# qianlim/CAPE

Hardware: NVIDIA B200
Metric: meshes/sec fwd+bwd CAPE-affineconv nz64 (higher is better)
Workload: dtype f32

## Files before the change

### cape_b200/_lib.py

```python
import ctypes as C
import os

_HERE = os.path.dirname(os.path.abspath(__file__))
LIB_PATH = os.environ.get("CAPE_B200_LIB") or os.path.join(_HERE, "libcape_b200.so")

MAX_TERMS = 8
EPI_LINEAR, EPI_AFFINE, EPI_SLOPE, EPI_DUALMASK = 0, 1, 2, 3
ACT_NONE, ACT_LEAKY, ACT_RELU = 0, 1, 2

f32p = C.c_void_p


class Term(C.Structure):
    _fields_ = [("src", C.c_void_p), ("op", C.c_int), ("F", C.c_int), ("src_rows", C.c_int),
                ("src_stride", C.c_int), ("w_stride", C.c_int), ("w2_stride", C.c_int), ("w", C.c_void_p), ("w2", C.c_void_p),
                ("wc", C.c_void_p), ("wc2", C.c_void_p), ("wT", C.c_void_p), ("w2T", C.c_void_p),
                ("wT_stride", C.c_int), ("w2T_stride", C.c_int), ("stash", C.c_void_p), ("stash_stride", C.c_int),
                ("wT_lo", C.c_void_p), ("w2T_lo", C.c_void_p)]


class ConvArgs(C.Structure):
    _fields_ = [("N", C.c_int), ("rows_out", C.c_int), ("ncols", C.c_int), ("nterms", C.c_int),
                ("terms", Term * MAX_TERMS), ("cond", C.c_void_p), ("C", C.c_int), ("epilogue", C.c_int),
                ("act", C.c_int), ("alpha", C.c_float), ("bias", C.c_void_p), ("bias_per_row", C.c_int),
# ... 29 lines not shown
                ("F", C.c_int), ("src_rows", C.c_int), ("src_stride", C.c_int), ("g", C.c_void_p),
                ("dw", C.c_void_p), ("dw_stride", C.c_int), ("accumulate", C.c_int), ("nops", C.c_int),
                ("ops", C.c_int * MAX_TERMS), ("dw_term_stride", C.c_int), ("dw_col_stride", C.c_int)]


SIGNATURES = {
    "cape_last_error": (C.c_char_p, []),
    "cape_abi_version": (C.c_int, []),
    "cape_launch_count": (C.c_int64, []),
    "cape_topology_create": (C.c_int, [C.c_int, C.POINTER(C.c_void_p)]),
    "cape_topology_destroy": (None, [C.c_void_p]),
    "cape_topology_add_operator": (C.c_int, [C.c_void_p, C.c_int, C.c_int, C.c_int, C.c_void_p, C.c_void_p]),
    "cape_topology_reserve_workspace": (C.c_int, [C.c_void_p, C.c_int64]),
    "cape_set_tensor_cores": (C.c_int, [C.c_int]),
    "cape_tensor_cores_enabled": (C.c_int, []),
    "cape_gemm_batch": (C.c_int, [C.c_void_p, C.c_int, C.c_void_p, C.c_int, C.c_void_p]),
    "cape_gemm_item_bytes": (C.c_int, []),
    "cape_gather_rows": (C.c_int, [C.c_void_p, C.c_int64, C.c_int, C.c_void_p, C.c_int, C.c_void_p, C.c_void_p]),
    "cape_weight_prep": (C.c_int, [C.c_void_p, C.c_int, C.c_int, C.c_void_p]),
    "cape_set_tuning": (C.c_int, [C.c_int, C.c_int]),
    "cape_cheb_fwd": (C.c_int, [C.c_void_p, C.POINTER(ConvArgs), C.c_void_p]),
    "cape_apply": (C.c_int, [C.c_void_p, C.POINTER(ApplyArgs), C.c_void_p]),
    "cape_cheb_dw": (C.c_int, [C.c_void_p, C.POINTER(DwArgs), C.c_void_p]),
    "cape_colsum": (C.c_int, [C.c_void_p, C.c_void_p, C.c_int, C.c_int, C.c_int, C.c_int, C.POINTER(C.c_int), C.c_int,
                              C.c_void_p, C.c_void_p]),
    "cape_gemm": (C.c_int, [C.c_void_p, C.c_int, C.c_int, C.c_int, C.c_void_p, C.c_int64, C.c_int64, C.c_void_p,
                            C.c_int64, C.c_int64, C.c_void_p, C.c_int64, C.c_void_p, C.c_int, C.c_float, C.c_float,
                            C.c_float, C.c_void_p]),
    "cape_resample": (C.c_int, [C.c_void_p, C.c_int, C.c_void_p, C.c_int, C.c_void_p, C.c_int, C.c_int, C.c_int, C.c_int,
                                C.c_int, C.c_void_p, C.c_int, C.c_void_p]),
    "cape_cheb_weight_transpose": (C.c_int, [C.c_void_p, C.c_int, C.c_int, C.c_int, C.c_void_p, C.c_void_p, C.c_void_p]),
    "cape_tf32_lo": (C.c_int, [C.c_void_p, C.c_void_p, C.c_int64, C.c_void_p]),
    "cape_act_bwd": (C.c_int, [C.c_void_p, C.c_void_p, C.c_void_p, C.c_int64, C.c_float, C.c_void_p]),
    "cape_axpy": (C.c_int, [C.c_void_p, C.c_void_p, C.c_float, C.c_int64, C.c_void_p]),
    "cape_vae_sample_fwd": (C.c_int, [C.c_void_p, C.c_void_p, C.c_void_p, C.c_void_p, C.c_int, C.c_int, C.c_int,
                                      C.c_void_p]),
    "cape_vae_sample_bwd": (C.c_int, [C.c_void_p, C.c_int, C.c_void_p, C.c_void_p, C.c_void_p, C.c_void_p,
                                      C.c_void_p, C.c_int, C.c_int, C.c_float, C.c_void_p]),
    "cape_recon_losses": (C.c_int, [C.c_void_p, C.c_int, C.c_void_p, C.c_void_p, C.c_int, C.c_int, C.c_float,
                                    C.c_float, C.c_int, C.c_void_p, C.c_void_p, C.c_int, C.c_void_p, C.c_void_p,
                                    C.c_void_p]),
    "cape_bce_logits": (C.c_int, [C.c_void_p, C.c_int64, C.c_float, C.c_float, C.c_void_p, C.c_void_p, C.c_void_p]),
    "cape_sumsq": (C.c_int, [C.c_void_p, C.c_int64, C.c_void_p, C.c_void_p]),
    "cape_sgd_clip_update": (C.c_int, [C.c_void_p, C.c_void_p, C.c_void_p, C.c_int64, C.c_void_p, C.c_float,
                                       C.c_void_p, C.c_float, C.c_void_p]),
    "cape_adam_clip_update": (C.c_int, [C.c_void_p, C.c_void_p, C.c_void_p, C.c_void_p, C.c_int64, C.c_void_p, C.c_float,
# ... 35 lines not shown
```

### cape_b200/csrc/dw_dense_tma.cu

```cuda
#include "common.cuh"
#include "ellconv_params.cuh"
#include "tc_common.cuh"

namespace cape {

namespace {

using namespace tc;

constexpr int DD_CONV_WARPS = 8;
constexpr int DD_CONV_THREADS = DD_CONV_WARPS * 32;
constexpr int DD_THREADS = DD_CONV_THREADS + 64;
constexpr int DD_KCH = 32;
constexpr int DD_A_TILE = 4 * 4096;
constexpr int DD_MAX_STAGES = 8;
constexpr int DD_SMEM_BUDGET = 212 * 1024;

struct DdParams {
  int ncols, F;
  long long total_rows, rows_per_split;
  float* out;
  long long out_rs;
  int nsplit, accumulate, ovec, lo_mode;
  int sah, sal, sgh, sgl;
  int budget;
};

template <int BN>
struct DdCfg {
  static constexpr int G_TILE = (BN / 32) * 4096;
  static constexpr int SMEM_BYTES = 1024 + DD_SMEM_BUDGET + 1024;
};

template <int BN>
void dd_plan(int nct, DdParams* p) {
  constexpr int GT = DdCfg<BN>::G_TILE;
  p->sal = 2; p->sgl = 2;
  int left = p->budget - 2 * DD_A_TILE - 2 * GT;
  int sah = nct >= 2 ? 3 : 2, sgh = 2;
  left -= sah * DD_A_TILE + sgh * GT;
  while (true) {
    const bool to_g = (sgh < DD_MAX_STAGES) && ((long long)sgh < (long long)sah * nct || sah >= DD_MAX_STAGES);
    const int cost = to_g ? GT : DD_A_TILE;
    if ((to_g ? sgh : sah) >= DD_MAX_STAGES || cost > left) break;
    left -= cost;
    if (to_g) ++sgh; else ++sah;
  }
  p->sah = sah; p->sgh = sgh;
// ... 40 lines not shown
  if (warp == DD_CONV_WARPS) {
    if (lane == 0) {
      for (int s = 0; s < DD_MAX_STAGES; ++s) {
        mbar_init(bar_ahf + 8 * s, 1); mbar_init(bar_ahe + 8 * s, 1);
        mbar_init(bar_alf + 8 * s, DD_CONV_WARPS); mbar_init(bar_ale + 8 * s, 1);
        mbar_init(bar_ghf + 8 * s, 1); mbar_init(bar_ghe + 8 * s, 1);
        mbar_init(bar_glf + 8 * s, DD_CONV_WARPS); mbar_init(bar_gle + 8 * s, 1);
      }
      mbar_init(bar_accum, 1);
      fence_mbar_init();
    }
    __syncwarp();
    tmem_alloc(smem_u32(tmem_slot), (uint32_t)tmem_cols);
  }
  tc_fence_before();
  __syncthreads();
  tc_fence_after();
  const uint32_t tmem_base = *tmem_slot;

  if (warp < DD_CONV_WARPS) {
    int ah = 0, al = 0, gh = 0, gl = 0;
    uint32_t pah = 0, pal = 0, pgh = 0, pgl = 0;
    const int mode = p.lo_mode;
    for (long long kc = 0; kc < nchunks; ++kc) {
      {
        mbar_wait(bar_ahf + 8 * ah, pah);
        mbar_wait(bar_ale + 8 * al, pal ^ 1);
        const char* hi = ahi_ring + (size_t)ah * DD_A_TILE;
        char* lo = alo_ring + (size_t)al * DD_A_TILE;
#pragma unroll
        for (int i = 0; i < DD_A_TILE / 16 / DD_CONV_THREADS; ++i) {
          if (i >= a_blocks) break;
          const int off = (i * DD_CONV_THREADS + tid) * 16;
          const float4 v = *reinterpret_cast<const float4*>(hi + off);
          *reinterpret_cast<float4*>(lo + off) =
              make_float4(lo_part(v.x, mode), lo_part(v.y, mode), lo_part(v.z, mode), lo_part(v.w, mode));
        }
        fence_proxy_async();
        __syncwarp();
        if (lane == 0) mbar_arrive(bar_alf + 8 * al);
        if (++ah == SAH) { ah = 0; pah ^= 1; }
        if (++al == SAL) { al = 0; pal ^= 1; }
      }
      for (int cs = 0; cs < nct; ++cs) {
        mbar_wait(bar_ghf + 8 * gh, pgh);
        mbar_wait(bar_gle + 8 * gl, pgl ^ 1);
        const char* hi = ghi_ring + (size_t)gh * Cfg::G_TILE;
        char* lo = glo_ring + (size_t)gl * Cfg::G_TILE;
#pragma unroll
        for (int i = 0; i < Cfg::G_TILE / 16 / DD_CONV_THREADS; ++i) {
          const int off = (i * DD_CONV_THREADS + tid) * 16;
          const float4 v = *reinterpret_cast<const float4*>(hi + off);
          *reinterpret_cast<float4*>(lo + off) =
              make_float4(lo_part(v.x, mode), lo_part(v.y, mode), lo_part(v.z, mode), lo_part(v.w, mode));
        }
        fence_proxy_async();
        __syncwarp();
        if (lane == 0) mbar_arrive(bar_glf + 8 * gl);
        if (++gh == SGH) { gh = 0; pgh ^= 1; }
        if (++gl == SGL) { gl = 0; pgl ^= 1; }
      }
    }

    mbar_wait(bar_accum, 0);
    tc_fence_after();
    const int quad = warp & 3, half = warp >> 2;
    const int f = ftile + quad * 32 + lane;
    const int cpw = p.ncols >> 1;
    const uint32_t taddr_row = tmem_base + ((uint32_t)(quad * 32) << 16);
    float* orow = p.out + (p.nsplit > 1 ? (size_t)blockIdx.y * p.F * p.out_rs : 0) + (size_t)f * p.out_rs;
#pragma unroll 1
    for (int g = 0; g < cpw / 16; ++g) {
      const int c0 = half * cpw + g * 16;
      float v[16];
      tmem_ld16(taddr_row + (uint32_t)c0, v);
      if (f >= p.F) continue;
      if (nchunks == 0) {
#pragma unroll
        for (int j = 0; j < 16; ++j) v[j] = 0.f;
      }
      if (p.nsplit == 1 && p.accumulate) {
#pragma unroll
        for (int j = 0; j < 16; ++j) orow[c0 + j] += v[j];
      } else if (p.ovec) {
#pragma unroll
// ... 132 lines not shown
int launch_dd(const CUtensorMap& ma, const CUtensorMap& mg, const DdParams& p, int ftiles, cudaStream_t st) {
  using Cfg = DdCfg<BN>;
  static bool configured = false;
  if (!configured) {
    CAPE_CHECK_CUDA(cudaFuncSetAttribute(dw_dense_kernel<BN>, cudaFuncAttributeMaxDynamicSharedMemorySize, Cfg::SMEM_BYTES));
    configured = true;
  }
  const int nct = (p.ncols + BN - 1) / BN;
  int tmem_cols = 32;
  while (tmem_cols < nct * BN) tmem_cols *= 2;
  DdParams q = p;
  q.budget = BN <= 64 ? 104 * 1024 : DD_SMEM_BUDGET;
  dd_plan<BN>(nct, &q);
  dim3 grid(ftiles, q.nsplit);
  dw_dense_kernel<BN><<<grid, DD_THREADS, 1024 + q.budget + 1024, st>>>(ma, mg, q, nct, tmem_cols);
  CAPE_CHECK_CUDA(cudaGetLastError());
  count_launches(1);
  return 1;
}

}

int launch_dw_dense_tma(const cape_topology* t, const cape_dw_args* a, const OpView& op, int* nsplit_out,
                        cudaStream_t st) {
  if (!tensor_cores_enabled() || g_tuning[1] == 1) return 0;
  if (op.idx != nullptr || a->src_rows != a->rows_out) return 0;
  if (a->ncols % 32 != 0 || a->ncols < 32 || a->ncols > 512) return 0;
  if (a->F % 4 != 0 || a->F < 32 || a->src_stride % 4 != 0 || !aligned16(a->src) || !aligned16(a->g)) return 0;
  const long long total_rows = (long long)a->N * a->rows_out;
  if (total_rows < 4096 || total_rows >= (1LL << 31)) return 0;
  CUtensorMap ma, mg;
  if (!make_map(&ma, a->src, a->F, total_rows, a->src_stride)) return 0;
  if (!make_map(&mg, a->g, a->ncols, total_rows, a->ncols)) return 0;
  DdParams p{};
  p.ncols = a->ncols; p.F = a->F; p.total_rows = total_rows; p.lo_mode = g_tuning[2];
  const int ftiles = (a->F + 127) / 128;
  const bool two_per_sm = a->ncols <= 64;
  long long nsplit = (two_per_sm ? 2 : 1) * t->sm_count / ftiles;
  if (nsplit < 1) nsplit = 1;
  if (total_rows / nsplit > 4096) nsplit *= 2;
  const long long max_by_rows = (total_rows + 255) / 256;
  if (nsplit > max_by_rows) nsplit = max_by_rows;
  const long long per = (long long)a->F * a->ncols * (long long)sizeof(float);
  if (nsplit > 1 && nsplit * per > t->workspace_bytes) nsplit = t->workspace_bytes / per;
  if (nsplit < 1) nsplit = 1;
  long long rps = (total_rows + nsplit - 1) / nsplit;
  rps = (rps + DD_KCH - 1) / DD_KCH * DD_KCH;
  nsplit = (total_rows + rps - 1) / rps;
  p.rows_per_split = rps; p.nsplit = (int)nsplit; p.accumulate = a->accumulate;
  if (nsplit == 1) { p.out = a->dw; p.out_rs = a->dw_stride; }
  else { p.out = (float*)t->workspace; p.out_rs = a->ncols; }
  p.ovec = (p.out_rs % 4 == 0) && aligned16(p.out);
  *nsplit_out = (int)nsplit;
  if (a->ncols % 256 == 0 && g_tuning[3] != 2) return launch_dd<256>(ma, mg, p, ftiles, st);
  if (a->ncols > 64) return launch_dd<128>(ma, mg, p, ftiles, st);
  if (a->ncols > 32) return launch_dd<64>(ma, mg, p, ftiles, st);
  return launch_dd<32>(ma, mg, p, ftiles, st);
}

}
```

### cape_b200/csrc/ellconv.cu

```cuda
#include "common.cuh"
#include "ellconv_params.cuh"

namespace cape {

__device__ __forceinline__ void gather_A(const TermDev& tm, int f0, const int* s_n, const int* s_r, int tid,
                                         float (&ra)[16]) {
  if (tm.vec) {
    const int l8 = tid & 7, rs = tid >> 3;
    const int f = f0 + l8 * 4;
#pragma unroll
    for (int i = 0; i < 4; ++i) {
      const int row = rs + 32 * i;
      const int n = s_n[row], r = s_r[row];
      float4 v = make_float4(0.f, 0.f, 0.f, 0.f);
      if (n >= 0 && f < tm.F) {
        const float* base = tm.src + (size_t)n * tm.src_rows * tm.src_stride + f;
        if (tm.op.idx == nullptr) {
          v = ldg4(base + (size_t)r * tm.src_stride);
        } else {
          ell_gather4(tm.op, r, base, (size_t)tm.src_stride, v);
        }
      }
      ra[4 * i + 0] = v.x; ra[4 * i + 1] = v.y; ra[4 * i + 2] = v.z; ra[4 * i + 3] = v.w;
    }
// ... 453 lines not shown
#pragma unroll 4
      for (int z = zl; z < nsplit; z += 32) s += ws[(size_t)z * total + e];
    }
    red[zl][el] = s;
    __syncthreads();
    if (zl == 0 && e < total) {
      s = 0.f;
#pragma unroll
      for (int k = 0; k < 32; ++k) s += red[k][el];
      const int q = (int)(e / ncols), c = (int)(e % ncols);
      float* o = dw + (size_t)(q % Fper) * dw_stride + (size_t)(q / Fper) * term_stride + (size_t)c * col_stride;
      *o = accumulate ? (*o + s) : s;
    }
    __syncthreads();
  }
}

constexpr int CS_MAXOPS = 4;
struct ColsumParams {
  const float* g;
  int N, rows, ncols, nops, rows_per_block, vec, gs;
  const float* coef[CS_MAXOPS];
  float* out;
};

__global__ void __launch_bounds__(256) colsum_kernel(const __grid_constant__ ColsumParams p) {
  __shared__ float red[CS_MAXOPS][256 * 4 / 32][33];
  const int n = blockIdx.y;
  const int r0 = blockIdx.x * p.rows_per_block;
  const int r1 = min(p.rows, r0 + p.rows_per_block);
  const float* gp = p.g + (size_t)n * p.rows * p.gs;
  if (p.vec) {
    const int cl = p.ncols >> 2;
    const int rl = 256 / cl;
    const int c4 = threadIdx.x % cl, ry = threadIdx.x / cl;
    float4 s[CS_MAXOPS];
#pragma unroll
    for (int j = 0; j < CS_MAXOPS; ++j) s[j] = make_float4(0.f, 0.f, 0.f, 0.f);
    if (ry < rl) {
      int r = r0 + ry;
      for (; r + 3 * rl < r1; r += 4 * rl) {
        const float* g0 = gp + (size_t)r * p.gs + c4 * 4;
        const size_t step = (size_t)rl * p.gs;
        const float4 v0 = ldg4(g0), v1 = ldg4(g0 + step), v2 = ldg4(g0 + 2 * step), v3 = ldg4(g0 + 3 * step);
#pragma unroll
        for (int j = 0; j < CS_MAXOPS; ++j)
          if (j < p.nops) {
            const float* cf = p.coef[j];
            const float k0 = cf ? __ldg(cf + r) : 1.f, k1 = cf ? __ldg(cf + r + rl) : 1.f;
            const float k2 = cf ? __ldg(cf + r + 2 * rl) : 1.f, k3 = cf ? __ldg(cf + r + 3 * rl) : 1.f;
            fma4(s[j], k0, v0); fma4(s[j], k1, v1); fma4(s[j], k2, v2); fma4(s[j], k3, v3);
          }
      }
      for (; r < r1; r += rl) {
        const float4 gv = ldg4(gp + (size_t)r * p.gs + c4 * 4);
#pragma unroll
        for (int j = 0; j < CS_MAXOPS; ++j)
          if (j < p.nops) fma4(s[j], p.coef[j] ? __ldg(p.coef[j] + r) : 1.f, gv);
      }
    }
    float* sm = &red[0][0][0];
    for (int j = 0; j < p.nops; ++j) {
      __syncthreads();
      if (ry < rl) *reinterpret_cast<float4*>(sm + ((size_t)ry * cl + c4) * 4) = s[j];
      __syncthreads();
      for (int c = threadIdx.x; c < p.ncols; c += 256) {
        float tot = 0.f;
        for (int k = 0; k < rl; ++k) tot += sm[((size_t)k * cl + (c >> 2)) * 4 + (c & 3)];
        atomicAdd(p.out + ((size_t)n * p.nops + j) * p.ncols + c, tot);
      }
    }
  } else {
    const int cx = threadIdx.x & 31, ry = threadIdx.x >> 5;
    for (int c0 = 0; c0 < p.ncols; c0 += 32) {
      const int c = c0 + cx;
      float s[CS_MAXOPS] = {0.f, 0.f, 0.f, 0.f};
      if (c < p.ncols)
        for (int r = r0 + ry; r < r1; r += 8) {
          const float gv = __ldg(gp + (size_t)r * p.gs + c);
#pragma unroll
          for (int j = 0; j < CS_MAXOPS; ++j)
            if (j < p.nops) s[j] = fmaf(p.coef[j] ? __ldg(p.coef[j] + r) : 1.f, gv, s[j]);
        }
      __syncthreads();
#pragma unroll
      for (int j = 0; j < CS_MAXOPS; ++j) red[j][ry][cx] = s[j];
      __syncthreads();
      if (ry == 0 && c < p.ncols)
        for (int j = 0; j < p.nops; ++j) {
          float tot = 0.f;
#pragma unroll
          for (int k = 0; k < 8; ++k) tot += red[j][k][cx];
          atomicAdd(p.out + ((size_t)n * p.nops + j) * p.ncols + c, tot);
        }
    }
  }
}

__global__ void __launch_bounds__(256) resample_kernel(OpView op, const float* __restrict__ x, int xs,
                                                       float* __restrict__ y, int ys, long long total_rows,
                                                       int rows_out, int rows_in, int F, int vec,
                                                       const float* __restrict__ cond, int C) {
  const long long warp = ((long long)blockIdx.x * blockDim.x + threadIdx.x) >> 5;
  const int lane = threadIdx.x & 31;
  if (warp >= total_rows) return;
  const int n = (int)(warp / rows_out), r = (int)(warp % rows_out);
  const float* base = x + (size_t)n * rows_in * xs;
  float* out = y + (size_t)warp * ys;
  if (vec) {
    for (int f = lane * 4; f < F; f += 128) {
      float4 v = make_float4(0.f, 0.f, 0.f, 0.f);
      if (op.idx == nullptr) v = ldg4(base + (size_t)r * xs + f);
      else ell_gather4(op, r, base + f, (size_t)xs, v);
      *reinterpret_cast<float4*>(out + f) = v;
    }
  } else {
// ... 120 lines not shown
      const TermDev& d = p.terms[i];
      if (!d.stash) continue;
      const long long blocks = (p.total_rows * 32 + 255) / 256;
      const int vec = d.vec && (d.stash_stride % 4 == 0);
      resample_kernel<<<(unsigned)blocks, 256, 0, st>>>(d.op, d.src, d.src_stride, d.stash, d.stash_stride, p.total_rows,
                                                        a->rows_out, d.src_rows, d.F, vec, nullptr, 0);
      CAPE_CHECK_CUDA(cudaGetLastError());
      cape::count_launches(1);
    }
  }
  dim3 grid((unsigned)((p.total_rows + BM - 1) / BM), (unsigned)((a->ncols + BNsel - 1) / BNsel));
  if (dual) {
    if (BNsel == 32) ellconv_kernel<32, true><<<grid, NT, 0, st>>>(p);
    else ellconv_kernel<64, true><<<grid, NT, 0, st>>>(p);
  } else {
    if (BNsel == 32) ellconv_kernel<32, false><<<grid, NT, 0, st>>>(p);
    else ellconv_kernel<64, false><<<grid, NT, 0, st>>>(p);
  }
  CAPE_CHECK_CUDA(cudaGetLastError());
  cape::count_launches(1);
  return 0;
}

static int dw_single(cape_topology* t, const cape_dw_args* a, void* stream);

extern "C" int cape_cheb_dw(cape_topology* t, const cape_dw_args* a, void* stream) {
  CAPE_REQUIRE(t && a, "null handle/args");
  CAPE_REQUIRE(a->N > 0 && a->rows_out > 0 && a->ncols > 0 && a->F > 0, "empty problem");
  CAPE_REQUIRE(a->src && a->g && a->dw, "null pointer");
  CAPE_REQUIRE(a->src_stride >= a->F && (a->dw_stride >= a->ncols || a->dw_col_stride > 1), "bad strides");
  if (a->nops <= 0) {
    CAPE_REQUIRE(a->dw_col_stride <= 1, "dw_col_stride needs the multi-term form (nops > 0)");
    return dw_single(t, a, stream);
  }
  CAPE_REQUIRE(a->nops <= CAPE_MAX_TERMS, "nops out of range");
  OpView ops[CAPE_MAX_TERMS];
  for (int j = 0; j < a->nops; ++j)
    if (get_op(t, a->ops[j], a->rows_out, a->src_rows, &ops[j]) != 0) return -1;
  int ns = 1;
  int rc = launch_thin_dw(t, a, ops, a->nops, &ns, (cudaStream_t)stream);
  if (rc < 0) return rc;
  if (rc == 1) {
    const long long total = (long long)a->nops * a->F * a->ncols;
    long long blocks = (total + 31) / 32;
    if (blocks > 8LL * t->sm_count) blocks = 8LL * t->sm_count;
    reduce_splits_kernel<<<(unsigned)blocks, 1024, 0, (cudaStream_t)stream>>>(
        (const float*)t->workspace, ns, a->nops * a->F, a->ncols, a->dw, a->dw_stride, a->accumulate, a->F,
        a->dw_term_stride, a->dw_col_stride > 0 ? a->dw_col_stride : 1);
    CAPE_CHECK_CUDA(cudaGetLastError());
    cape::count_launches(1);
    return 0;
  }
  CAPE_REQUIRE(a->dw_col_stride <= 1, "dw_col_stride is only implemented for thin inputs (F <= 4, ncols 32..256)");
  for (int j = 0; j < a->nops; ++j) {
    cape_dw_args b = *a;
    b.nops = 0; b.op = a->ops[j]; b.dw = a->dw + (size_t)j * a->dw_term_stride;
    rc = dw_single(t, &b, stream);
    if (rc != 0) return rc;
  }
  return 0;
}

static int dw_single(cape_topology* t, const cape_dw_args* a, void* stream) {
  DwParams p{};
  if (get_op(t, a->op, a->rows_out, a->src_rows, &p.op) != 0) return -1;
  {
    int ns = 1;
    bool always_reduce = false;
    int rc = launch_thin_dw(t, a, &p.op, 1, &ns, (cudaStream_t)stream);
    if (rc < 0) return rc;
    if (rc == 1) always_reduce = true;
    else rc = launch_dw_dense_tma(t, a, p.op, &ns, (cudaStream_t)stream);
    if (rc < 0) return rc;
    if (rc == 0) rc = launch_ellconv_dw_tc(t, a, p.op, &ns, (cudaStream_t)stream);
    if (rc < 0) return rc;
    if (rc == 1) {
      if (ns > 1 || always_reduce) {
        const long long total = (long long)a->F * a->ncols;
        long long blocks = (total + 31) / 32;
        if (blocks > 8LL * t->sm_count) blocks = 8LL * t->sm_count;
        reduce_splits_kernel<<<(unsigned)blocks, 1024, 0, (cudaStream_t)stream>>>((const float*)t->workspace, ns, a->F,
                                                                                 a->ncols, a->dw, a->dw_stride,
                                                                                 a->accumulate, a->F, 0, 1);
        CAPE_CHECK_CUDA(cudaGetLastError());
        cape::count_launches(1);
      }
      return 0;
    }
  }
  p.N = a->N; p.rows_out = a->rows_out; p.ncols = a->ncols;
  p.total_rows = (long long)a->N * a->rows_out;
  p.src = a->src; p.F = a->F; p.src_rows = a->src_rows; p.src_stride = a->src_stride;
  p.g = a->g;
  p.vec = (a->F % 4 == 0) && (a->src_stride % 4 == 0) && aligned16(a->src);
  p.gvec = (a->ncols % 4 == 0) && aligned16(a->g);
// ... 8 lines not shown
  long long rps = (p.total_rows + nsplit - 1) / nsplit;
  rps = (rps + DW_BR - 1) / DW_BR * DW_BR;
  nsplit = (p.total_rows + rps - 1) / rps;
  p.rows_per_split = rps; p.nsplit = (int)nsplit; p.accumulate = a->accumulate;
  cudaStream_t st = (cudaStream_t)stream;
  if (nsplit == 1) { p.out = a->dw; p.out_rs = a->dw_stride; }
  else { p.out = (float*)t->workspace; p.out_rs = a->ncols; }
  dim3 grid(ftiles, ctiles, (unsigned)nsplit);
  ellconv_dw_kernel<<<grid, NT, 0, st>>>(p);
  CAPE_CHECK_CUDA(cudaGetLastError());
  cape::count_launches(1);
  if (nsplit > 1) {
    const long long total = (long long)a->F * a->ncols;
    long long blocks = (total + 31) / 32;
    if (blocks > 8LL * t->sm_count) blocks = 8LL * t->sm_count;
    reduce_splits_kernel<<<(unsigned)blocks, 1024, 0, st>>>((const float*)t->workspace, (int)nsplit, a->F, a->ncols, a->dw,
                                                  a->dw_stride, a->accumulate, a->F, 0, 1);
    CAPE_CHECK_CUDA(cudaGetLastError());
  cape::count_launches(1);
  }
  return 0;
}

extern "C" int cape_colsum(cape_topology* t, const float* g, int g_stride, int N, int rows, int ncols, const int* ops,
                           int nops, float* out, void* stream) {
  CAPE_REQUIRE(t && g && out, "null pointer");
  CAPE_REQUIRE(nops >= 1 && nops <= CS_MAXOPS, "nops out of range");
  CAPE_REQUIRE(N > 0 && rows > 0 && ncols > 0, "empty problem");
  ColsumParams p{};
  CAPE_REQUIRE(g_stride >= ncols, "bad g_stride");
  p.g = g; p.N = N; p.rows = rows; p.ncols = ncols; p.nops = nops; p.out = out; p.gs = g_stride;
  for (int j = 0; j < nops; ++j) {
    const int op = ops ? ops[j] : -1;
    if (op < 0) { p.coef[j] = nullptr; continue; }
    CAPE_REQUIRE(op < (int)t->ops.size(), "operator id out of range");
    CAPE_REQUIRE(t->ops[op].rows_out == rows, "colsum: operator rows mismatch");
    p.coef[j] = t->ops[op].rowsum;
  }
  p.vec = (ncols % 4 == 0) && (g_stride % 4 == 0) && ncols <= 512 && (256 % (ncols / 4) == 0) && aligned16(g);
  int rblocks = (4 * t->sm_count + N - 1) / N;
  if (rblocks < 1) rblocks = 1;
  int rpb = (rows + rblocks - 1) / rblocks;
  if (rpb < 64) rpb = 64;
  rblocks = (rows + rpb - 1) / rpb;
  p.rows_per_block = rpb;
  CAPE_REQUIRE(N <= 65535, "grid too large");
  dim3 grid(rblocks, N);
  colsum_kernel<<<grid, 256, 0, (cudaStream_t)stream>>>(p);
  CAPE_CHECK_CUDA(cudaGetLastError());
  cape::count_launches(1);
  return 0;
}
```

### cape_b200/csrc/ellconv_params.cuh

```cuda
#pragma once
#include "common.cuh"

namespace cape {

constexpr int BM = 128;
constexpr int BK = 32;
constexpr int NT = 256;
constexpr int AS_STRIDE = BK + 4;
constexpr int MAX_SLOTS = 2 * CAPE_MAX_TERMS;

struct TermDev {
  const float* src;
  OpView op;
  int F, src_rows, src_stride, w_stride, w2_stride;
  const float* w;
  const float* w2;
  const float* wT;
  const float* w2T;
  int wT_stride, w2T_stride;
  int vec;
  const float* wT_lo;
  const float* w2T_lo;
  float* stash;
  int stash_stride;
// ... 13 lines not shown
  float alpha;
  const float* bias;
  int bias_per_row;
  const float* aux;
  float* out;
  float* out2;
  int wvec, ovec;
  int split_rn;
  int precise;
};


int launch_gemm_tc(const cape_topology* t, const ConvParams& p, bool dual, cudaStream_t st);
int launch_ellconv_tc(const cape_topology* t, const ConvParams& p, bool dual, cudaStream_t st);
bool tensor_cores_enabled();
int launch_thin_fwd(const cape_topology* t, const ConvParams& p, bool dual, cudaStream_t st);
int launch_thinout_fwd(const cape_topology* t, const ConvParams& p, bool dual, cudaStream_t st);
int launch_thin_dw(const cape_topology* t, const cape_dw_args* a, const OpView* ops, int nops, int* nsplit_out,
                   cudaStream_t st);
int launch_ellconv_dw_tc(const cape_topology* t, const cape_dw_args* a, const OpView& op, int* nsplit_out,
                         cudaStream_t st);

int launch_dw_dense_tma(const cape_topology* t, const cape_dw_args* a, const OpView& op, int* nsplit_out,
                        cudaStream_t st);
extern int g_tuning[32];

}
```

### cape_b200/engine.py

```python
import ctypes as C

import numpy as np
import scipy.sparse as sp
import torch

from . import _lib
from . import topology as topo
from ._lib import (ACT_LEAKY, ACT_NONE, ACT_RELU, EPI_AFFINE, EPI_DUALMASK, EPI_LINEAR, EPI_SLOPE, ApplyArgs, ConvArgs,
                   DwArgs, GemmItem, WPrep, check)

LEAKY_ALPHA = 0.2

PROFILE = None
TRACE = bool(int(__import__("os").environ.get("CAPE_TRACE", "0")))


class _Prof:
    def __init__(self, family, tag):
        self.on = PROFILE is not None and tag is not None
        self.family, self.tag = family, tag

    def __enter__(self):
        if self.on:
            self.e0 = torch.cuda.Event(enable_timing=True)
# ... 223 lines not shown
    def flush(self):
        if not self.pending:
            return
        key = tuple(self.pending)
        n = len(key)
        tab = self.tables.get(key)
        if tab is None:
            arr = (GemmItem * n)()
            for d, it in zip(arr, key):
                (d.a, d.a_rs, d.a_cs, d.b, d.b_rs, d.b_cs, d.c, d.c_rs, d.M, d.N, d.K, d.alpha, d.beta) = it
            tab = torch.empty(n * self.item_bytes, dtype=torch.uint8, device=self.tp.device)
            torch.cuda.synchronize()
            check(self.tp.lib.cape_gemm_batch(C.cast(arr, C.c_void_p), n, C.c_void_p(tab.data_ptr()), 0, _stream()))
            self.tables[key] = tab
        check(self.tp.lib.cape_gemm_batch(None, n, C.c_void_p(tab.data_ptr()), self.blocks_per_item, _stream()))
        self.pending = []


def tensor_cores_enabled(tp):
    return bool(tp.lib.cape_tensor_cores_enabled())


def cheb_dw(tp, N, rows_out, ncols, src, op, F, src_rows, src_stride, g, dw, dw_stride, accumulate=False, tag=None,
            dw_term_stride=0, dw_col_stride=0):
    a = DwArgs()
    a.N, a.rows_out, a.ncols = N, rows_out, ncols
    if isinstance(op, (list, tuple)):
        a.nops, a.dw_term_stride, a.dw_col_stride = len(op), dw_term_stride, dw_col_stride
        for j, o in enumerate(op):
            a.ops[j] = o
        op = op[0]
    a.src, a.op, a.F, a.src_rows, a.src_stride = src.data_ptr(), op, F, src_rows, src_stride
    a.g, a.dw, a.dw_stride, a.accumulate = g.data_ptr(), dw.data_ptr(), dw_stride, 1 if accumulate else 0
    with _Prof("ellconv_dw", tag):
        check(tp.lib.cape_cheb_dw(tp.h, C.byref(a), _stream()))


def colsum(tp, g, N, rows, ncols, ops, out, g_stride=None):
    arr = (C.c_int * len(ops))(*ops)
    check(tp.lib.cape_colsum(tp.h, _ptr(g), ncols if g_stride is None else g_stride, N, rows, ncols, arr, len(ops),
                             _ptr(out), _stream()))


def weight_transpose(tp, w, Fin, K, Fout, wt, wt_lo=None):
    check(tp.lib.cape_cheb_weight_transpose(_ptr(w), Fin, K, Fout, _ptr(wt), _ptr(wt_lo), _stream()))


def tf32_lo(tp, x, lo):
    check(tp.lib.cape_tf32_lo(_ptr(_f32(x)), _ptr(_f32(lo)), x.numel(), _stream()))


def act_bwd(tp, dy, y, g, alpha=LEAKY_ALPHA):
    check(tp.lib.cape_act_bwd(_ptr(dy), _ptr(y), _ptr(g), dy.numel(), alpha, _stream()))


def axpy(tp, y, x, a):
    check(tp.lib.cape_axpy(_ptr(y), _ptr(x), float(a), y.numel(), _stream()))

# ... 18 lines not shown
```

### cape_b200/network.py

```python
import math
import os

import numpy as np
import torch

from . import _lib
from . import engine as E
from . import topology as topo
from .engine import (ACT_LEAKY, ACT_NONE, EPI_AFFINE, EPI_DUALMASK, EPI_LINEAR, EPI_SLOPE, ConvSite, Topology,
                     act_bwd, axpy, cheb_call, cheb_dw, colsum, gemm)
from .params import init_params, is_d_param, is_g_param, param_specs


ADAM_BETA1, ADAM_BETA2, ADAM_EPS = float(np.float32(0.9)), float(np.float32(0.999)), 1e-8


def _pad4(n):
    return (n + 3) // 4 * 4


class ParamStore:

    def __init__(self, specs, names, device):
        self.names = list(names)
# ... 230 lines not shown
                     w_stride=K * Fout, wT=self.Wt[k], wT_stride=F, wT_lo=self.Wt_lo[k])
            if C:
                t["wc"] = self.W3[F:, k, :]
            if basis and s.ops[k] != -1:
                t.update(src=self.stash_a[k][:N], op=-1, src_rows=s.rows_out, src_stride=F)
            elif self.stash_a[k] is not None:
                t["stash"], t["stash_stride"] = self.stash_a[k][:N], F
            if self.affine and k == 0:
                t["w2"], t["w2_stride"] = self.Wa2, Fout
                t["w2T"], t["w2T_stride"], t["w2T_lo"] = self.Wt[K], F, self.Wt_lo[K]
                if C:
                    t["wc2"] = self.Wa2[F:]
            terms.append(t)
        cheb_call(self.tp, N, s.rows_out, Fout, terms, out, out2=out2, cond=ycat if C else None,
                  epilogue=EPI_AFFINE if self.affine else EPI_LINEAR, act=self.act, bias=self.bias,
                  bias_per_row=self.bias_per_row, tag=tag, precise=self.precise)

    def bwd(self, x, ycat, g, g_aff=None, dx=None, dx2=None, dx_epi=EPI_LINEAR, dx_aux=None, dx_alpha=E.LEAKY_ALPHA,
            dycat=None, want_dw=True, cs_slot=0):
        tp, s, F, C, K, Fout = self.tp, self.site, self.F, self.C, self.K, self.Fout
        N = g.shape[0]
        sx = x.shape[2]
        mode = self.dw_mode if (want_dw and (self.dw_mode != "gside" or dx is not None)) else "gather"
        if want_dw and mode == "aside":
            nl = K + (1 if self.affine else 0)
            tg = (self.name + ":dW", self.alg_bytes(N, "dW") / nl)

            def dw_aside(tp):
                for k in range(K):
                    B = self.stash_a[k]
                    if B is None:
                        cheb_dw(tp, N, s.rows_out, Fout, x, -1, F, s.rows_in, sx, g, self.gW3[:, k, :], K * Fout, tag=tg)
                    else:
                        cheb_dw(tp, N, s.rows_out, Fout, B[:N], -1, F, s.rows_out, F, g, self.gW3[:, k, :], K * Fout,
                                tag=tg)
                if self.affine:
                    B = self.stash_a[0]
                    if B is None:
                        cheb_dw(tp, N, s.rows_out, Fout, x, -1, F, s.rows_in, sx, g_aff, self.gWa2, Fout, tag=tg)
                    else:
                        cheb_dw(tp, N, s.rows_out, Fout, B[:N], -1, F, s.rows_out, F, g_aff, self.gWa2, Fout, tag=tg)
            self.net.run_dw(dw_aside)
        elif (want_dw and mode == "gather" and Fout <= 4 and not self.affine and F in (32, 64, 128, 256) and sx == F
              and K <= 4):
            cheb_dw(tp, N, s.rows_in, F, g, list(s.opsT), Fout, s.rows_out, Fout, x, self.gW3, 1,
                    tag=(self.name + ":dW", self.alg_bytes(N, "dW")), dw_term_stride=Fout, dw_col_stride=K * Fout)
        elif want_dw and mode == "gather":
            nl = (1 if F <= 4 else K) + (1 if self.affine else 0)
            tg = (self.name + ":dW", self.alg_bytes(N, "dW") / nl)
            if F <= 4:
                cheb_dw(tp, N, s.rows_out, Fout, x, list(s.ops), F, s.rows_in, sx, g, self.gW3, K * Fout, tag=tg,
                        dw_term_stride=Fout)
            for k in range(K if F > 4 else 0):
                cheb_dw(tp, N, s.rows_out, Fout, x, s.ops[k], F, s.rows_in, sx, g, self.gW3[:, k, :], K * Fout, tag=tg)
            if self.affine:
                cheb_dw(tp, N, s.rows_out, Fout, x, s.ops[0], F, s.rows_in, sx, g_aff, self.gWa2, Fout, tag=tg)
        has_bias = self.bias is not None and not self.bias_per_row and want_dw
        if (has_bias or C) and len(self.cs_ops):
            cs = self.net.arena.get(self.cs_id[cs_slot])[:N]
            nops = len(self.cs_ops)
            if nops <= 4:
                self.net.run_glue(lambda: colsum(tp, g, N, s.rows_out, Fout, self.cs_ops, cs))
            else:
                for o in range(0, nops, 4):
                    self._colsum_chunk(g, N, cs, o)
            sg = self.net.small.add
            if has_bias:
                sg(self.net.ones[:, :N], cs[:, 0, :], self.gbias.view(1, Fout))
            if C:
                for k in range(K):
                    dq = cs[:, self.cs_cond0 + k, :]
                    if want_dw:
                        sg(ycat.t(), dq, self.gW3[F:, k, :])
                    if dycat is not None:
                        sg(dq, self.W3[F:, k, :].t(), dycat, beta=1.0)
        if self.affine and C:
            csa = self.net.arena.get(self.csa_id)[:N]
            self.net.run_glue(lambda: colsum(tp, g_aff, N, s.rows_out, Fout, [s.ops[0]], csa))
            if want_dw:
                self.net.small.add(ycat.t(), csa[:, 0, :], self.gWa2[F:])
            if dycat is not None:
                self.net.small.add(csa[:, 0, :], self.Wa2[F:].t(), dycat, beta=1.0)
        if self.bias_per_row and want_dw:
            self.net.small.add(self.net.ones[:, :N], g.view(N, s.rows_out * Fout), self.gbias.view(1, s.rows_out * Fout))
        if dx is not None:
            assert self.need_dx
            gs = want_dw and mode == "gside"
            dtag = (self.name + ":dx", self.alg_bytes(N, "dx"))
            sub = lambda what: (self.name + ":dx/" + what, 0)
            if self.dx_mode == "contract" and self._split():
                Z = self.net.scratch[: N * s.rows_out * K * F].view(N, s.rows_out, K * F)
                cheb_call(tp, N, s.rows_out, K * F,
                          [dict(src=g, op=-1, F=Fout, src_rows=s.rows_out, src_stride=Fout, w=None, w_stride=0,
                                wT=self.Wk.view(K * F, Fout), wT_stride=Fout, wT_lo=self.Wk_lo.view(K * F, Fout))],
                          Z, plain_only=True, tag=sub("project"))
                E.apply_call(tp, N, s.rows_in, F,
                             [dict(src=Z[:, :, k * F:], op=s.opsT[k], src_rows=s.rows_out, src_stride=K * F)
                              for k in range(K)], dx, out2=dx2, epilogue=dx_epi, aux=dx_aux, alpha=dx_alpha, tag=dtag)
            else:
                basis = gs and self.dx_mode == "basis" and self._split()
                terms = []
# ... 6 lines not shown
                for k in range(K):
                    t = dict(src=g, op=s.opsT[k], F=Fout, src_rows=s.rows_out, src_stride=Fout,
                             w=self.Wt[k], w_stride=F, wT=self.W3[:, k, :], wT_stride=K * Fout,
                             wT_lo=self.W3_lo[:, k, :])
                    if gs and self.stash_g[k] is not None:
                        t["stash"], t["stash_stride"] = self.stash_g[k][:N], self.stash_g[k].stride(1)
                    terms.append(t)
                if basis:
                    for i, t in enumerate(terms):
                        if t["op"] == -1:
                            continue
                        H, hs = t.pop("stash"), t.pop("stash_stride")
                        E.apply_call(tp, N, s.rows_in, Fout,
                                     [dict(src=t["src"], op=t["op"], src_rows=s.rows_out, src_stride=Fout)], H,
                                     out_stride=hs, tag=sub("narrow%d" % i))
                        t.update(src=H, op=-1, src_rows=s.rows_in, src_stride=hs)
                cheb_call(tp, N, s.rows_in, F, terms, dx, out2=dx2, epilogue=dx_epi, aux=dx_aux, alpha=dx_alpha, tag=dtag)
            if gs:
                nl = (1 if self.g_merged else K) + (1 if self.affine else 0)
                tg = (self.name + ":dW", self.alg_bytes(N, "dW") / nl)

                def dw_gside(tp):
                    if self.g_merged:
                        cheb_dw(tp, N, s.rows_in, K * Fout, x, -1, F, s.rows_in, sx, self.Hg[:N], self.gW3, K * Fout, tag=tg)
                    else:
                        for k in range(K):
                            H = g if self.stash_g[k] is None else self.stash_g[k][:N]
                            cheb_dw(tp, N, s.rows_in, Fout, x, -1, F, s.rows_in, sx, H, self.gW3[:, k, :], K * Fout,
                                    tag=tg)
                    if self.affine:
                        Ha = g_aff if self.stash_ga is None else self.stash_ga[:N]
                        cheb_dw(tp, N, s.rows_in, Fout, x, -1, F, s.rows_in, sx, Ha, self.gWa2, Fout, tag=tg)
                self.net.run_dw(dw_gside)

    def _colsum_chunk(self, g, N, cs, o):
        ops = self.cs_ops[o:o + 4]
        tmp = torch.zeros(N, len(ops), self.Fout, device=g.device)
        colsum(self.tp, g, N, self.site.rows_out, self.Fout, ops, tmp)
        cs[:, o:o + len(ops), :] = tmp


class Dense:

    def __init__(self, net, W, b, gW, gb, act=ACT_NONE, name=""):
        self.net, self.tp, self.name = net, net.tp, name
        self.W, self.b, self.gW, self.gb, self.act = W, b, gW, gb, act

    def fwd(self, x, out):
        M, K = x.shape
        Nn = self.W.shape[1]
        gemm(self.tp, x, self.W, out, bias=self.b, act=self.act,
             tag=(self.name + ":fwd", 4 * (M * (K + Nn) + K * Nn)))

    def bwd(self, x, out, dout, gtmp=None, dx=None, dx_beta=0.0, want_dw=True):
        g = dout
# ... 293 lines not shown
        out.update(self.PD.export(self.PD.grad))
        return out

    def set_params(self, vals):
        self.PG.load(vals)
        self.PD.load(vals)
        self.prep_weights()

    def all_layers(self):
        dec = self.dec if self.affine else [l for b in self.dec for l in b.layers()]
        return self.enc + [self.enc_1x1, self.dec_1x1] + dec + [self.dec_out] + self.disc + [self.disc_pred]

    def run_dw(self, fn):
        if not self.async_dw or E.PROFILE is not None:
            fn(self.tp)
            return
        ev = torch.cuda.Event()
        ev.record()
        self.dw_stream.wait_event(ev)
        with torch.cuda.stream(self.dw_stream):
            fn(self.tp_dw)
        self._dw_pending = True

    def run_glue(self, fn):
        if self.side_glue:
            self.run_dw(lambda _tp: fn())
        else:
            fn()

    def join_dw(self):
        if self._dw_pending:
            torch.cuda.current_stream().wait_stream(self.dw_stream)
            self._dw_pending = False

    def lo_of(self, t):
        r = self.PG.lo_of(t)
        return r if r is not None else self.PD.lo_of(t)

    def prep_weights(self):
        E.tf32_lo(self.tp, self.PG.flat, self.PG.lo)
        E.tf32_lo(self.tp, self.PD.flat, self.PD.lo)
        self.wprep.run()

    def scratch_req(self, nfloats):
        self._scratch_need = max(getattr(self, "_scratch_need", 4), int(nfloats))

# ... 345 lines not shown
```

### include/cape_b200.h

```cpp
#ifndef CAPE_B200_H
#define CAPE_B200_H

#include <stdint.h>

#ifdef __cplusplus
extern "C" {
#endif

#define CAPE_ABI_VERSION 3
#define CAPE_MAX_TERMS 8

typedef struct cape_topology cape_topology;

const char* cape_last_error(void);
int cape_abi_version(void);
int64_t cape_launch_count(void);

int cape_topology_create(int device, cape_topology** out);
void cape_topology_destroy(cape_topology* t);
int cape_topology_add_operator(cape_topology* t, int rows_out, int rows_in, int width,
                               const int32_t* idx_host, const float* w_host);
int cape_topology_reserve_workspace(cape_topology* t, int64_t bytes);

typedef struct {
// ... 73 lines not shown
} cape_apply_args;
int cape_apply(cape_topology* t, const cape_apply_args* a, void* stream);

int cape_set_tuning(int key, int value);

int cape_set_tensor_cores(int enable);
int cape_tensor_cores_enabled(void);

int cape_cheb_fwd(cape_topology* t, const cape_conv_args* a, void* stream);

typedef struct {
  int N, rows_out, ncols;
  const float* src; int op; int F; int src_rows; int src_stride;
  const float* g;
  float* dw; int dw_stride;
  int accumulate;
  int nops;
  int ops[CAPE_MAX_TERMS];
  int dw_term_stride;
  int dw_col_stride;
} cape_dw_args;
int cape_cheb_dw(cape_topology* t, const cape_dw_args* a, void* stream);

int cape_colsum(cape_topology* t, const float* g, int g_stride, int N, int rows, int ncols,
                const int* ops, int nops, float* out, void* stream);

int cape_gemm(cape_topology* t, int M, int N, int K,
              const float* a, int64_t a_rs, int64_t a_cs,
              const float* b, int64_t b_rs, int64_t b_cs,
              float* c, int64_t c_rs,
              const float* bias, int act, float leaky_alpha, float alpha, float beta, void* stream);

typedef struct {
  const float* a; int64_t a_rs, a_cs;
  const float* b; int64_t b_rs, b_cs;
  float* c; int64_t c_rs;
  int M, N, K;
  float alpha, beta;
} cape_gemm_item;
int cape_gemm_batch(const cape_gemm_item* items_host, int n, void* table_device, int blocks_per_item, void* stream);
int cape_gemm_item_bytes(void);

int cape_resample(cape_topology* t, int op, const float* x, int x_stride, float* y, int y_stride, int N, int rows_out,
                  int rows_in, int F, const float* cond, int C, void* stream);

int cape_cheb_weight_transpose(const float* w, int Fin, int K, int Fout, float* wt, float* wt_lo, void* stream);
// ... 48 lines not shown
```

Baseline: 5108.

## Fuse gradient column-sum into dense TMA weight-gradient kernel

Adds a cape_cheb_dw_colsum entry point. In the dense TMA dW kernel, block 0 accumulates per-mesh column sums of the gradient tile it already reads while splitting it into hi/lo parts, then flushes them with atomics. The network layer routes bias and conditioning column sums through this path when the dW result feeds the glue stream, which skips separate colsum launches and the extra pass over g. It adds register pressure and atomics to the dW kernel, and falls back to a separate colsum launch when the fused path does not apply.

```diff
diff --git a/cape_b200/_lib.py b/cape_b200/_lib.py
--- a/cape_b200/_lib.py
+++ b/cape_b200/_lib.py
@@ -75,6 +75,7 @@
     "cape_cheb_fwd": (C.c_int, [C.c_void_p, C.POINTER(ConvArgs), C.c_void_p]),
     "cape_apply": (C.c_int, [C.c_void_p, C.POINTER(ApplyArgs), C.c_void_p]),
     "cape_cheb_dw": (C.c_int, [C.c_void_p, C.POINTER(DwArgs), C.c_void_p]),
+    "cape_cheb_dw_colsum": (C.c_int, [C.c_void_p, C.POINTER(DwArgs), C.c_void_p, C.c_int64, C.c_void_p]),
     "cape_colsum": (C.c_int, [C.c_void_p, C.c_void_p, C.c_int, C.c_int, C.c_int, C.c_int, C.POINTER(C.c_int), C.c_int,
                               C.c_void_p, C.c_void_p]),
     "cape_gemm": (C.c_int, [C.c_void_p, C.c_int, C.c_int, C.c_int, C.c_void_p, C.c_int64, C.c_int64, C.c_void_p,
diff --git a/cape_b200/csrc/dw_dense_tma.cu b/cape_b200/csrc/dw_dense_tma.cu
--- a/cape_b200/csrc/dw_dense_tma.cu
+++ b/cape_b200/csrc/dw_dense_tma.cu
@@ -24,6 +24,9 @@
   int nsplit, accumulate, ovec, lo_mode;
   int sah, sal, sgh, sgl;
   int budget;
+  float* cs;
+  long long cs_stride;
+  int cs_rows;
 };
 
 template <int BN>
@@ -110,7 +113,32 @@
     int ah = 0, al = 0, gh = 0, gl = 0;
     uint32_t pah = 0, pal = 0, pgh = 0, pgl = 0;
     const int mode = p.lo_mode;
+    const bool do_cs = p.cs != nullptr && blockIdx.x == 0;
+    const int cs_row = (tid >> 5) * 4 + ((tid >> 3) & 3);
+    const int cs_col = (((((tid >> 1) & 3) ^ ((tid >> 3) & 3)) << 1) | (tid & 1)) * 4;
+    float4 csum[BN / 32];
+#pragma unroll
+    for (int i = 0; i < BN / 32; ++i) csum[i] = make_float4(0.f, 0.f, 0.f, 0.f);
+    long long cs_n = (rbeg + cs_row) / (do_cs ? p.cs_rows : 1), cs_next = (cs_n + 1) * p.cs_rows;
+    auto cs_flush = [&]() {
+      if (cs_n * p.cs_rows >= p.total_rows) return;
+      float* o = p.cs + cs_n * p.cs_stride + cs_col;
+#pragma unroll
+      for (int i = 0; i < BN / 32; ++i) {
+        atomicAdd(o + i * 32, csum[i].x); atomicAdd(o + i * 32 + 1, csum[i].y);
+        atomicAdd(o + i * 32 + 2, csum[i].z); atomicAdd(o + i * 32 + 3, csum[i].w);
+        csum[i] = make_float4(0.f, 0.f, 0.f, 0.f);
+      }
+    };
     for (long long kc = 0; kc < nchunks; ++kc) {
+      if (do_cs) {
+        const long long R = rbeg + kc * DD_KCH + cs_row;
+        if (R >= cs_next) {
+          cs_flush();
+          cs_n = R / p.cs_rows;
+          cs_next = (cs_n + 1) * p.cs_rows;
+        }
+      }
       {
         mbar_wait(bar_ahf + 8 * ah, pah);
         mbar_wait(bar_ale + 8 * al, pal ^ 1);
@@ -141,6 +169,7 @@
           const float4 v = *reinterpret_cast<const float4*>(hi + off);
           *reinterpret_cast<float4*>(lo + off) =
               make_float4(lo_part(v.x, mode), lo_part(v.y, mode), lo_part(v.z, mode), lo_part(v.w, mode));
+          if (do_cs) { csum[i].x += v.x; csum[i].y += v.y; csum[i].z += v.z; csum[i].w += v.w; }
         }
         fence_proxy_async();
         __syncwarp();
@@ -149,6 +178,8 @@
         if (++gl == SGL) { gl = 0; pgl ^= 1; }
       }
     }
+
+    if (do_cs) cs_flush();
 
     mbar_wait(bar_accum, 0);
     tc_fence_after();
@@ -327,7 +358,7 @@
 }
 
 int launch_dw_dense_tma(const cape_topology* t, const cape_dw_args* a, const OpView& op, int* nsplit_out,
-                        cudaStream_t st) {
+                        float* cs, long long cs_stride, bool* cs_done, cudaStream_t st) {
   if (!tensor_cores_enabled() || g_tuning[1] == 1) return 0;
   if (op.idx != nullptr || a->src_rows != a->rows_out) return 0;
   if (a->ncols % 32 != 0 || a->ncols < 32 || a->ncols > 512) return 0;
@@ -357,6 +388,11 @@
   else { p.out = (float*)t->workspace; p.out_rs = a->ncols; }
   p.ovec = (p.out_rs % 4 == 0) && aligned16(p.out);
   *nsplit_out = (int)nsplit;
+  const int bn = (a->ncols % 256 == 0 && g_tuning[3] != 2) ? 256 : a->ncols > 64 ? 128 : a->ncols > 32 ? 64 : 32;
+  if (cs != nullptr && a->ncols <= bn) {
+    p.cs = cs; p.cs_stride = cs_stride; p.cs_rows = a->rows_out;
+    *cs_done = true;
+  }
   if (a->ncols % 256 == 0 && g_tuning[3] != 2) return launch_dd<256>(ma, mg, p, ftiles, st);
   if (a->ncols > 64) return launch_dd<128>(ma, mg, p, ftiles, st);
   if (a->ncols > 32) return launch_dd<64>(ma, mg, p, ftiles, st);
diff --git a/cape_b200/csrc/ellconv.cu b/cape_b200/csrc/ellconv.cu
--- a/cape_b200/csrc/ellconv.cu
+++ b/cape_b200/csrc/ellconv.cu
@@ -499,6 +499,7 @@
   int N, rows, ncols, nops, rows_per_block, vec, gs;
   const float* coef[CS_MAXOPS];
   float* out;
+  long long os;
 };
 
 __global__ void __launch_bounds__(256) colsum_kernel(const __grid_constant__ ColsumParams p) {
@@ -544,7 +545,7 @@
       for (int c = threadIdx.x; c < p.ncols; c += 256) {
         float tot = 0.f;
         for (int k = 0; k < rl; ++k) tot += sm[((size_t)k * cl + (c >> 2)) * 4 + (c & 3)];
-        atomicAdd(p.out + ((size_t)n * p.nops + j) * p.ncols + c, tot);
+        atomicAdd(p.out + (size_t)n * p.os + (size_t)j * p.ncols + c, tot);
       }
     }
   } else {
@@ -568,7 +569,7 @@
           float tot = 0.f;
 #pragma unroll
           for (int k = 0; k < 8; ++k) tot += red[j][k][cx];
-          atomicAdd(p.out + ((size_t)n * p.nops + j) * p.ncols + c, tot);
+          atomicAdd(p.out + (size_t)n * p.os + (size_t)j * p.ncols + c, tot);
         }
     }
   }
@@ -735,13 +736,19 @@
   return 0;
 }
 
-static int dw_single(cape_topology* t, const cape_dw_args* a, void* stream);
-
-extern "C" int cape_cheb_dw(cape_topology* t, const cape_dw_args* a, void* stream) {
+static int dw_single(cape_topology* t, const cape_dw_args* a, void* stream, float* cs = nullptr,
+                     long long cs_stride = 0, bool* cs_done = nullptr);
+
+static int check_dw_args(const cape_topology* t, const cape_dw_args* a) {
   CAPE_REQUIRE(t && a, "null handle/args");
   CAPE_REQUIRE(a->N > 0 && a->rows_out > 0 && a->ncols > 0 && a->F > 0, "empty problem");
   CAPE_REQUIRE(a->src && a->g && a->dw, "null pointer");
   CAPE_REQUIRE(a->src_stride >= a->F && (a->dw_stride >= a->ncols || a->dw_col_stride > 1), "bad strides");
+  return 0;
+}
+
+extern "C" int cape_cheb_dw(cape_topology* t, const cape_dw_args* a, void* stream) {
+  if (check_dw_args(t, a) != 0) return -1;
   if (a->nops <= 0) {
     CAPE_REQUIRE(a->dw_col_stride <= 1, "dw_col_stride needs the multi-term form (nops > 0)");
     return dw_single(t, a, stream);
@@ -774,7 +781,8 @@
   return 0;
 }
 
-static int dw_single(cape_topology* t, const cape_dw_args* a, void* stream) {
+static int dw_single(cape_topology* t, const cape_dw_args* a, void* stream, float* cs, long long cs_stride,
+                     bool* cs_done) {
   DwParams p{};
   if (get_op(t, a->op, a->rows_out, a->src_rows, &p.op) != 0) return -1;
   {
@@ -783,7 +791,7 @@
     int rc = launch_thin_dw(t, a, &p.op, 1, &ns, (cudaStream_t)stream);
     if (rc < 0) return rc;
     if (rc == 1) always_reduce = true;
-    else rc = launch_dw_dense_tma(t, a, p.op, &ns, (cudaStream_t)stream);
+    else rc = launch_dw_dense_tma(t, a, p.op, &ns, cs, cs_stride, cs_done, (cudaStream_t)stream);
     if (rc < 0) return rc;
     if (rc == 0) rc = launch_ellconv_dw_tc(t, a, p.op, &ns, (cudaStream_t)stream);
     if (rc < 0) return rc;
@@ -838,14 +846,14 @@
   return 0;
 }
 
-extern "C" int cape_colsum(cape_topology* t, const float* g, int g_stride, int N, int rows, int ncols, const int* ops,
-                           int nops, float* out, void* stream) {
+static int colsum_launch(cape_topology* t, const float* g, int g_stride, int N, int rows, int ncols, const int* ops,
+                         int nops, float* out, long long out_stride, void* stream) {
   CAPE_REQUIRE(t && g && out, "null pointer");
   CAPE_REQUIRE(nops >= 1 && nops <= CS_MAXOPS, "nops out of range");
   CAPE_REQUIRE(N > 0 && rows > 0 && ncols > 0, "empty problem");
   ColsumParams p{};
   CAPE_REQUIRE(g_stride >= ncols, "bad g_stride");
-  p.g = g; p.N = N; p.rows = rows; p.ncols = ncols; p.nops = nops; p.out = out; p.gs = g_stride;
+  p.g = g; p.N = N; p.rows = rows; p.ncols = ncols; p.nops = nops; p.out = out; p.os = out_stride; p.gs = g_stride;
   for (int j = 0; j < nops; ++j) {
     const int op = ops ? ops[j] : -1;
     if (op < 0) { p.coef[j] = nullptr; continue; }
@@ -867,3 +875,20 @@
   cape::count_launches(1);
   return 0;
 }
+
+extern "C" int cape_colsum(cape_topology* t, const float* g, int g_stride, int N, int rows, int ncols, const int* ops,
+                           int nops, float* out, void* stream) {
+  return colsum_launch(t, g, g_stride, N, rows, ncols, ops, nops, out, (long long)nops * ncols, stream);
+}
+
+extern "C" int cape_cheb_dw_colsum(cape_topology* t, const cape_dw_args* a, float* colsum, int64_t colsum_stride,
+                                   void* stream) {
+  if (check_dw_args(t, a) != 0) return -1;
+  CAPE_REQUIRE(colsum != nullptr, "null colsum");
+  CAPE_REQUIRE(a->nops <= 0 && a->dw_col_stride <= 1, "cape_cheb_dw_colsum takes the single-term form (nops = 0)");
+  CAPE_REQUIRE(colsum_stride >= a->ncols, "bad colsum_stride");
+  bool done = false;
+  const int rc = dw_single(t, a, stream, colsum, colsum_stride, &done);
+  if (rc != 0 || done) return rc;
+  return colsum_launch(t, a->g, a->ncols, a->N, a->rows_out, a->ncols, nullptr, 1, colsum, colsum_stride, stream);
+}
diff --git a/cape_b200/csrc/ellconv_params.cuh b/cape_b200/csrc/ellconv_params.cuh
--- a/cape_b200/csrc/ellconv_params.cuh
+++ b/cape_b200/csrc/ellconv_params.cuh
@@ -59,7 +59,7 @@
                          cudaStream_t st);
 
 int launch_dw_dense_tma(const cape_topology* t, const cape_dw_args* a, const OpView& op, int* nsplit_out,
-                        cudaStream_t st);
+                        float* cs, long long cs_stride, bool* cs_done, cudaStream_t st);
 extern int g_tuning[32];
 
 }
diff --git a/cape_b200/engine.py b/cape_b200/engine.py
--- a/cape_b200/engine.py
+++ b/cape_b200/engine.py
@@ -269,7 +269,7 @@
 
 
 def cheb_dw(tp, N, rows_out, ncols, src, op, F, src_rows, src_stride, g, dw, dw_stride, accumulate=False, tag=None,
-            dw_term_stride=0, dw_col_stride=0):
+            dw_term_stride=0, dw_col_stride=0, colsum=None):
     a = DwArgs()
     a.N, a.rows_out, a.ncols = N, rows_out, ncols
     if isinstance(op, (list, tuple)):
@@ -280,7 +280,11 @@
     a.src, a.op, a.F, a.src_rows, a.src_stride = src.data_ptr(), op, F, src_rows, src_stride
     a.g, a.dw, a.dw_stride, a.accumulate = g.data_ptr(), dw.data_ptr(), dw_stride, 1 if accumulate else 0
     with _Prof("ellconv_dw", tag):
-        check(tp.lib.cape_cheb_dw(tp.h, C.byref(a), _stream()))
+        if colsum is None:
+            check(tp.lib.cape_cheb_dw(tp.h, C.byref(a), _stream()))
+        else:
+            assert colsum.stride(1) == 1 and colsum.shape[0] >= N and colsum.shape[1] >= ncols
+            check(tp.lib.cape_cheb_dw_colsum(tp.h, C.byref(a), _ptr(colsum), colsum.stride(0), _stream()))
 
 
 def colsum(tp, g, N, rows, ncols, ops, out, g_stride=None):
diff --git a/cape_b200/network.py b/cape_b200/network.py
--- a/cape_b200/network.py
+++ b/cape_b200/network.py
@@ -276,6 +276,13 @@
         N = g.shape[0]
         sx = x.shape[2]
         mode = self.dw_mode if (want_dw and (self.dw_mode != "gside" or dx is not None)) else "gather"
+        has_bias = self.bias is not None and not self.bias_per_row and want_dw
+        cs = self.net.arena.get(self.cs_id[cs_slot])[:N] if (has_bias or C) and len(self.cs_ops) else None
+        csa = self.net.arena.get(self.csa_id)[:N] if (self.affine and C) else None
+        fuse = want_dw and self.net.dw_feeds_glue()
+        cs_dw = cs is not None and fuse and ((mode == "aside" and self.cs_ops == [-1])
+                                             or (mode == "gside" and self.cs_ops == list(s.ops)))
+        csa_dw = csa is not None and fuse and mode == "gside"
         if want_dw and mode == "aside":
             nl = K + (1 if self.affine else 0)
             tg = (self.name + ":dW", self.alg_bytes(N, "dW") / nl)
@@ -283,11 +290,13 @@
             def dw_aside(tp):
                 for k in range(K):
                     B = self.stash_a[k]
+                    bsum = cs[:, 0, :] if cs_dw and k == 0 else None
                     if B is None:
-                        cheb_dw(tp, N, s.rows_out, Fout, x, -1, F, s.rows_in, sx, g, self.gW3[:, k, :], K * Fout, tag=tg)
+                        cheb_dw(tp, N, s.rows_out, Fout, x, -1, F, s.rows_in, sx, g, self.gW3[:, k, :], K * Fout, tag=tg,
+                                colsum=bsum)
                     else:
                         cheb_dw(tp, N, s.rows_out, Fout, B[:N], -1, F, s.rows_out, F, g, self.gW3[:, k, :], K * Fout,
-                                tag=tg)
+                                tag=tg, colsum=bsum)
                 if self.affine:
                     B = self.stash_a[0]
                     if B is None:
@@ -309,13 +318,11 @@
                 cheb_dw(tp, N, s.rows_out, Fout, x, s.ops[k], F, s.rows_in, sx, g, self.gW3[:, k, :], K * Fout, tag=tg)
             if self.affine:
                 cheb_dw(tp, N, s.rows_out, Fout, x, s.ops[0], F, s.rows_in, sx, g_aff, self.gWa2, Fout, tag=tg)
-        has_bias = self.bias is not None and not self.bias_per_row and want_dw
-        if (has_bias or C) and len(self.cs_ops):
-            cs = self.net.arena.get(self.cs_id[cs_slot])[:N]
+        if cs is not None:
             nops = len(self.cs_ops)
-            if nops <= 4:
+            if not cs_dw and nops <= 4:
                 self.net.run_glue(lambda: colsum(tp, g, N, s.rows_out, Fout, self.cs_ops, cs))
-            else:
+            elif not cs_dw:
                 for o in range(0, nops, 4):
                     self._colsum_chunk(g, N, cs, o)
             sg = self.net.small.add
@@ -328,9 +335,9 @@
                         sg(ycat.t(), dq, self.gW3[F:, k, :])
                     if dycat is not None:
                         sg(dq, self.W3[F:, k, :].t(), dycat, beta=1.0)
-        if self.affine and C:
-            csa = self.net.arena.get(self.csa_id)[:N]
-            self.net.run_glue(lambda: colsum(tp, g_aff, N, s.rows_out, Fout, [s.ops[0]], csa))
+        if csa is not None:
+            if not csa_dw:
+                self.net.run_glue(lambda: colsum(tp, g_aff, N, s.rows_out, Fout, [s.ops[0]], csa))
             if want_dw:
                 self.net.small.add(ycat.t(), csa[:, 0, :], self.gWa2[F:])
             if dycat is not None:
@@ -383,15 +390,17 @@
 
                 def dw_gside(tp):
                     if self.g_merged:
-                        cheb_dw(tp, N, s.rows_in, K * Fout, x, -1, F, s.rows_in, sx, self.Hg[:N], self.gW3, K * Fout, tag=tg)
+                        cheb_dw(tp, N, s.rows_in, K * Fout, x, -1, F, s.rows_in, sx, self.Hg[:N], self.gW3, K * Fout, tag=tg,
+                                colsum=cs.view(N, K * Fout) if cs_dw else None)
                     else:
                         for k in range(K):
                             H = g if self.stash_g[k] is None else self.stash_g[k][:N]
                             cheb_dw(tp, N, s.rows_in, Fout, x, -1, F, s.rows_in, sx, H, self.gW3[:, k, :], K * Fout,
-                                    tag=tg)
+                                    tag=tg, colsum=cs[:, k, :] if cs_dw else None)
                     if self.affine:
                         Ha = g_aff if self.stash_ga is None else self.stash_ga[:N]
-                        cheb_dw(tp, N, s.rows_in, Fout, x, -1, F, s.rows_in, sx, Ha, self.gWa2, Fout, tag=tg)
+                        cheb_dw(tp, N, s.rows_in, Fout, x, -1, F, s.rows_in, sx, Ha, self.gWa2, Fout, tag=tg,
+                                colsum=csa[:, 0, :] if csa_dw else None)
                 self.net.run_dw(dw_gside)
 
     def _colsum_chunk(self, g, N, cs, o):
@@ -731,6 +740,9 @@
             fn(self.tp_dw)
         self._dw_pending = True
 
+    def dw_feeds_glue(self):
+        return self.side_glue or not self.async_dw or E.PROFILE is not None
+
     def run_glue(self, fn):
         if self.side_glue:
             self.run_dw(lambda _tp: fn())
diff --git a/include/cape_b200.h b/include/cape_b200.h
--- a/include/cape_b200.h
+++ b/include/cape_b200.h
@@ -119,6 +119,8 @@
 } cape_dw_args;
 int cape_cheb_dw(cape_topology* t, const cape_dw_args* a, void* stream);
 
+int cape_cheb_dw_colsum(cape_topology* t, const cape_dw_args* a, float* colsum, int64_t colsum_stride, void* stream);
+
 int cape_colsum(cape_topology* t, const float* g, int g_stride, int N, int rows, int ncols,
                 const int* ops, int nops, float* out, void* stream);
 
```

Result: faster. 5170 (median of 6 runs) (+1.2%).
